# thunlp/OpenMatch

Hardware: NVIDIA H100
Metric: queries/sec top-1000 over 8.8M x 768 corpus (higher is better)
Workload: dtype f16

## Files before the change

### openmatch_b200/csrc/scan_epilogue.cuh

```cuda
#pragma once
#include <cuda_fp16.h>
#include <string.h>

#include <type_traits>

#include "gemm.cuh"

namespace om {

__host__ __device__ __forceinline__ uint32_t f32_orderable(float s) {
  s = s + 0.0f;
#ifdef __CUDA_ARCH__
  uint32_t u = __float_as_uint(s);
#else
  uint32_t u;
  memcpy(&u, &s, 4);
#endif
  return (u & 0x80000000u) ? ~u : (u | 0x80000000u);
}
__host__ __device__ __forceinline__ float f32_from_orderable(uint32_t u) {
  u = (u & 0x80000000u) ? (u & 0x7fffffffu) : ~u;
#ifdef __CUDA_ARCH__
  return __uint_as_float(u);
#else
  float s;
  memcpy(&s, &u, 4);
  return s;
#endif
}
__host__ __device__ __forceinline__ unsigned long long make_key(float s, uint32_t row) {
  return (static_cast<unsigned long long>(f32_orderable(s)) << 32) | static_cast<unsigned long long>(0xffffffffu - row);
}
__host__ __device__ __forceinline__ uint32_t key_row(unsigned long long k) {
  return 0xffffffffu - static_cast<uint32_t>(k & 0xffffffffull);
}
__host__ __device__ __forceinline__ float key_score(unsigned long long k) {
  return f32_from_orderable(static_cast<uint32_t>(k >> 32));
}

constexpr int kStashThreads = 32 * kGemmEpiWarps;

template <int N>
using SurvivorMask = std::conditional_t<N == 64, unsigned long long, uint32_t>;
__device__ __forceinline__ int mask_popc(uint32_t m) { return __popc(m); }
__device__ __forceinline__ int mask_popc(unsigned long long m) { return __popcll(m); }
__device__ __forceinline__ int mask_ffs(uint32_t m) { return __ffs(m); }
__device__ __forceinline__ int mask_ffs(unsigned long long m) { return __ffsll(static_cast<long long>(m)); }

template <int N, int BIT = 1>
__device__ __forceinline__ float pick(const float (&v)[N], int i) {
  if constexpr (N == 1) {
    return v[0];
  } else {
    float a[N / 2];
#pragma unroll
    for (int j = 0; j < N / 2; ++j) a[j] = (i & BIT) ? v[2 * j + 1] : v[2 * j];
    return pick<N / 2, 2 * BIT>(a, i);
  }
}

template <int N>
__device__ __forceinline__ SurvivorMask<N> survivors(const float (&v)[N], float t) {
  float mx = fmaxf(v[0], v[1]);
#pragma unroll
  for (int i = 2; i < N; i += 2) mx = fmaxf(mx, fmaxf(v[i], v[i + 1]));
  if (!(mx > t)) return 0;
  SurvivorMask<N> mask = 0;
#pragma unroll
  for (int w = 0; w < N / 32; ++w) {
    uint32_t m = 0;
#pragma unroll
    for (int i = 0; i < 32; ++i) m |= (v[32 * w + i] > t ? 1u : 0u) << i;
    mask |= static_cast<SurvivorMask<N>>(m) << (32 * w);
  }
  return mask;
}

template <int S, int N, class Col>
__device__ __forceinline__ int park(const float (&v)[N], SurvivorMask<N> mask, Col col, int k, unsigned long long* stash,
                                    int row, unsigned long long* cand, int* count, int* overflow, int C,
                                    uint32_t row_base) {
  const int n = mask_popc(mask);
  int pos = 0;
  if (k + n > S) {
    pos = atomicAdd(count + row, k + n - S);
    if (pos + (k + n - S) > C) *overflow = 1;
  }
  unsigned long long* mine = cand + static_cast<size_t>(row) * C;
  int idx = k;
#pragma unroll 1
  while (mask) {
    const int i = mask_ffs(mask) - 1;
    mask &= mask - 1;
    const unsigned long long key = make_key(pick(v, i), row_base + static_cast<uint32_t>(col(i)));
    if (idx < S)
      stash[idx * kStashThreads] = key;
    else if (pos + idx - S < C)
      mine[pos + idx - S] = key;
    ++idx;
  }
  return idx < S ? idx : S;
}

template <int N, class Col>
__device__ __forceinline__ SurvivorMask<N> allowed(SurvivorMask<N> mask, const uint32_t* allow, uint32_t row_base, Col col) {
  SurvivorMask<N> keep = 0;
#pragma unroll 1
  while (mask) {
    const int i = mask_ffs(mask) - 1;
    const SurvivorMask<N> bit = static_cast<SurvivorMask<N>>(1) << i;
    mask &= ~bit;
    const uint32_t r = row_base + static_cast<uint32_t>(col(i));
    if ((__ldg(allow + (r >> 5)) >> (r & 31)) & 1u) keep |= bit;
  }
  return keep;
}

__device__ __forceinline__ void drain_stash(const unsigned long long* stash, int n, unsigned long long* list, int pos,
                                            int C, int* overflow) {
  for (int j = 0; j < n; ++j)
    if (pos + j < C) list[pos + j] = stash[j * kStashThreads];
  if (n > 0 && pos + n > C) *overflow = 1;
}

constexpr int kFragStash = 4;
constexpr int kFragStashBytes = 2 * 2 * kFragStash * kStashThreads * 8;

template <int COLS, bool ALLOW = false>
struct FragFilter {
  unsigned long long* stash;
  unsigned long long* cand;
  int* count;
  int* overflow;
  int C;
  uint32_t row_base;
  int lane;
  const uint32_t* allow = nullptr;
  int buf = 0;
  int p_n[2] = {0, 0}, p_excl[2] = {0, 0}, p_pos[2] = {0, 0}, p_row = 0, p_buf = 0;

  __device__ __forceinline__ int col(int i) const { return 8 * (i >> 1) + 2 * (lane & 3) + (i & 1); }

  template <int H>
  __device__ __forceinline__ int filter_row(const float (&acc)[2 * COLS], float t, int row, int col0, int lim,
                                            unsigned long long* sb) const {
    float v[COLS];
#pragma unroll
    for (int i = 0; i < COLS; ++i) v[i] = acc[4 * (i >> 1) + 2 * H + (i & 1)];
    SurvivorMask<COLS> mask = survivors(v, t);
    if (!mask) return 0;
    if (lim < 4 * COLS) {
#pragma unroll 1
      for (int i = 0; i < COLS; ++i)
        if (col(i) >= lim) mask &= ~(static_cast<SurvivorMask<COLS>>(1) << i);
    }
    if constexpr (ALLOW) mask = allowed<COLS>(mask, allow, row_base, [&](int i) { return col0 + col(i); });
    return park<kFragStash>(v, mask, [&](int i) { return col0 + col(i); }, 0, sb, row, cand, count, overflow, C,
                            row_base);
  }

  __device__ __forceinline__ void drain() {
    if (!__any_sync(0xffffffffu, (p_n[0] | p_n[1]) != 0)) return;
    const unsigned long long* s = stash + p_buf * (2 * kFragStash * kStashThreads);
#pragma unroll
    for (int h = 0; h < 2; ++h)
      drain_stash(s + h * kFragStash * kStashThreads, p_n[h], cand + static_cast<size_t>(p_row + 8 * h) * C,
                  __shfl_sync(0xffffffffu, p_pos[h], lane & ~3) + p_excl[h], C, overflow);
    p_n[0] = p_n[1] = 0;
  }

  __device__ __forceinline__ void tile(const float (&acc)[2 * COLS], float t0, float t1, int row0, int col0, int n_cols) {
    drain();
    const int lim = n_cols - col0;
    unsigned long long* sb = stash + buf * (2 * kFragStash * kStashThreads);
    const int k[2] = {filter_row<0>(acc, t0, row0, col0, lim, sb),
                      filter_row<1>(acc, t1, row0 + 8, col0, lim, sb + kFragStash * kStashThreads)};
    if (!__any_sync(0xffffffffu, (k[0] | k[1]) != 0)) return;
#pragma unroll
    for (int h = 0; h < 2; ++h) {
      int x = k[h];
      int y = __shfl_up_sync(0xffffffffu, x, 1, 4);
      if ((lane & 3) >= 1) x += y;
      y = __shfl_up_sync(0xffffffffu, x, 2, 4);
      if ((lane & 3) >= 2) x += y;
      const int n = __shfl_sync(0xffffffffu, x, lane | 3);
      if ((lane & 3) == 0 && n > 0) p_pos[h] = atomicAdd(count + row0 + 8 * h, n);
      p_n[h] = k[h];
      p_excl[h] = x - k[h];
    }
    p_row = row0;
    p_buf = buf;
    buf ^= 1;
  }
};

template <bool ALLOW>
struct ScanAllow {};
template <>
struct ScanAllow<true> {
  const uint32_t* allow;
};
template <bool DENSE, bool ALLOW = false>
struct EpiScan : ScanAllow<ALLOW> {
  static_assert(!(DENSE && ALLOW), "a filtered first round runs as a threshold round at -inf");
  const float* thr;
  unsigned long long* cand;
  int* count;
  int* overflow;
  int nq, n_cols, C;
  uint32_t row_base;
  static constexpr bool kPrefetch = false;
  static constexpr int kStash = 8;
  __host__ __device__ static constexpr int smem_bytes(int) { return DENSE ? 0 : 2 * kStash * kStashThreads * 8; }
  struct State {
    float t;
    int k, tid, buf;
    unsigned long long* stash;
    int p_n, p_pos, p_row, p_buf;
  };
  __device__ __forceinline__ void bind(State& s, uint8_t* smem, int epi_tid) const {
    s.stash = reinterpret_cast<unsigned long long*>(smem);
    s.tid = epi_tid;
    s.buf = 0;
    s.p_n = 0;
  }
  __device__ __forceinline__ void finish(State& s) const { drain(s); }
  __device__ __forceinline__ void begin(State& s, int row, int, int) const {
    s.t = (row < nq && !DENSE) ? thr[row] : __int_as_float(0x7f800000);
    s.k = 0;
    if constexpr (DENSE) {
      s.p_n = 0;
      s.buf = 0;
    }
  }
  __device__ __forceinline__ unsigned long long* slot0(const State& s, int buf) const {
    return s.stash + static_cast<size_t>(buf) * kStash * kStashThreads + s.tid;
  }
  __device__ __forceinline__ void drain(State& s) const {
    if (s.p_n > 0) {
      drain_stash(slot0(s, s.p_buf), s.p_n, cand + static_cast<size_t>(s.p_row) * C, s.p_pos, C, overflow);
      s.p_n = 0;
    }
  }
  __device__ __forceinline__ void end(State& s, int row) const {
    if constexpr (DENSE) return;
    drain(s);
    if (s.k > 0) {
      s.p_pos = atomicAdd(count + row, s.k);
      s.p_n = s.k;
      s.p_row = row;
      s.p_buf = s.buf;
      s.buf ^= 1;
    }
  }
  __device__ __forceinline__ void chunk(State& s, int row, int col0, const float (&v)[32]) const {
    if (row >= nq || col0 >= n_cols) return;
    if constexpr (DENSE) {
      unsigned long long* mine = cand + static_cast<size_t>(row) * C;
      if (col0 + 32 <= n_cols) {
#pragma unroll
        for (int i = 0; i < 32; i += 2) {
          ulonglong2 kk;
          kk.x = make_key(v[i], row_base + col0 + i);
          kk.y = make_key(v[i + 1], row_base + col0 + i + 1);
          *reinterpret_cast<ulonglong2*>(mine + col0 + i) = kk;
        }
      } else {
#pragma unroll
        for (int i = 0; i < 32; ++i)
          if (col0 + i < n_cols) mine[col0 + i] = make_key(v[i], row_base + col0 + i);
      }
      return;
    }
    uint32_t mask = survivors(v, s.t);
    if (!mask) return;
    const int lim = n_cols - col0;
    if (lim < 32) mask &= (1u << lim) - 1u;
    if constexpr (ALLOW) mask = allowed<32>(mask, this->allow, row_base + col0, [](int i) { return i; });
    s.k = park<kStash>(v, mask, [&](int i) { return col0 + i; }, s.k, slot0(s, s.buf), row, cand, count, overflow, C,
                       row_base);
  }
};

static inline cudaError_t launch_scan_core(bool dense, const uint32_t* allow, const __half* Q, int64_t ldq, const __half* X,
                                           int64_t ldx, int nq, int n_cols, int K, const float* thr,
                                           unsigned long long* cand, int* count, int* overflow, int C, uint32_t row_base,
                                           int num_sms, cudaStream_t stream) {
  auto launch = [&](const auto& epi) {
    return launch_gemm<128, 3, true, std::decay_t<decltype(epi)>, true>(Q, ldq, X, ldx, nq, n_cols, K, epi, num_sms, stream,
                                                                       true);
  };
  if (dense) return launch(EpiScan<true>{{}, thr, cand, count, overflow, nq, n_cols, C, row_base});
  if (allow) return launch(EpiScan<false, true>{{allow}, thr, cand, count, overflow, nq, n_cols, C, row_base});
  return launch(EpiScan<false>{{}, thr, cand, count, overflow, nq, n_cols, C, row_base});
}

}
```

### openmatch_b200/csrc/scan_gemm.cuh

```cuda
#pragma once
#include <cuda_fp16.h>

#include <type_traits>

#include "scan_epilogue.cuh"

namespace om {

constexpr int kScanBlockN = 256;
constexpr int kScanStages = 3;
constexpr int kScanABytes = kBlockM * kBlockK * 2;
constexpr int kScanBBytes = kScanBlockN * kBlockK * 2;
constexpr int kScanStageBytes = kScanABytes + kScanBBytes;
constexpr int kScanConsumers = kStashThreads;
constexpr int kScanStashOffset = kScanStages * kScanStageBytes;
constexpr int kScanBarOffset = kScanStashOffset + kFragStashBytes;
constexpr int kScanSmemBytes = kScanBarOffset + 2 * kScanStages * 8 + 1024;
static_assert(kScanSmemBytes <= 232448, "scan ring + stash exceed the 227 KB of shared memory an H100 block may use");

template <int CQ, int CX>
struct ScanCluster {
  static_assert((CQ == 2 || CQ == 4) && (CX == 1 || CX == 2), "scan cluster shapes: CQ in {2, 4}, CX in {1, 2}");
  static constexpr int kSize = CQ * CX;
  static constexpr int kShare = CQ + CX - 1;
  static constexpr int kQRows = kBlockM / CX;
  static constexpr int kXRows = kScanBlockN / CQ;
  static constexpr int kEmptyArrivals = kShare * (kScanConsumers / 32);
  __device__ static uint32_t peer_rank(uint32_t rank, int j) {
    const uint32_t a = rank % CQ, b = rank / CQ;
    if (j < CQ - 1) {
      const uint32_t o = static_cast<uint32_t>(j);
      return (o < a ? o : o + 1) + CQ * b;
    }
    const uint32_t o = static_cast<uint32_t>(j - (CQ - 1));
    return a + CQ * (o < b ? o : o + 1);
  }
  __device__ static uint16_t q_mask(uint32_t rank) {
    uint32_t m = 0;
#pragma unroll
    for (int b = 0; b < CX; ++b) m |= 1u << (rank % CQ + CQ * b);
    return static_cast<uint16_t>(m);
  }
  __device__ static uint16_t x_mask(uint32_t rank) {
    return static_cast<uint16_t>(((1u << CQ) - 1u) << (CQ * (rank / CQ)));
  }
};

template <int CQ, int CX, bool ALLOW>
__global__ void __launch_bounds__(kGemmProducerThreads + kScanConsumers, 1)
scan_wide_kernel(const __grid_constant__ CUtensorMap tmQ, const __grid_constant__ CUtensorMap tmX, int K,
                 const float* __restrict__ thr, unsigned long long* cand, int* count, int* overflow, int nq, int n_cols,
                 int C, uint32_t row_base, const uint32_t* __restrict__ allow) {
  using Cl = ScanCluster<CQ, CX>;
  extern __shared__ uint8_t smem_raw[];
  uint8_t* smem = reinterpret_cast<uint8_t*>((reinterpret_cast<uintptr_t>(smem_raw) + 1023) & ~uintptr_t(1023));
  unsigned long long* stash = reinterpret_cast<unsigned long long*>(smem + kScanStashOffset);
  uint64_t* full_bar = reinterpret_cast<uint64_t*>(smem + kScanBarOffset);
  uint64_t* empty_bar = full_bar + kScanStages;
  const uint32_t rank = cluster_ctarank();
  const int qa = static_cast<int>(rank % CQ), xb = static_cast<int>(rank / CQ);
  const int warp = __shfl_sync(0xffffffffu, static_cast<int>(threadIdx.x >> 5), 0);
  const int lane = static_cast<int>(threadIdx.x & 31);

  if (warp == 0 && lane == 0) {
    tma_prefetch_desc(&tmQ);
    tma_prefetch_desc(&tmX);
  }
  if (warp == 1 && lane == 0) {
    ring_init(full_bar, empty_bar, kScanStages, Cl::kEmptyArrivals);
    fence_barrier_init();
  }
  cluster_sync_all();

  const int qgroups = (nq + CQ * kBlockM - 1) / (CQ * kBlockM);
  const int num_tiles = qgroups * ((n_cols + CX * kScanBlockN - 1) / (CX * kScanBlockN));
  const int num_k = (K + kBlockK - 1) / kBlockK;

  if (warp < 4) {
    setmaxnreg_dec<40>();
    if (warp == 0 && lane == 0) {
      const uint16_t qmask = Cl::q_mask(rank), xmask = Cl::x_mask(rank);
      Ring<kScanStages> ring;
      for (int tile = static_cast<int>(cluster_id_x()); tile < num_tiles; tile += static_cast<int>(cluster_count_x())) {
        const int m_blk = (tile % qgroups) * CQ + qa;
        const int n_blk = (tile / qgroups) * CX + xb;
        for (int kb = 0; kb < num_k; ++kb) {
          uint64_t* bar = ring_acquire_tx(full_bar, empty_bar, ring, kScanStageBytes, 30);
          uint8_t* sa = smem + ring.stage * kScanStageBytes;
          if constexpr (CX == 1)
            tma_load_2d(sa, &tmQ, bar, kb * kBlockK, m_blk * kBlockM);
          else
            tma_load_2d_multicast(sa + xb * (Cl::kQRows * kBlockK * 2), &tmQ, bar, kb * kBlockK,
                                  m_blk * kBlockM + xb * Cl::kQRows, qmask);
          tma_load_2d_multicast(sa + kScanABytes + qa * (Cl::kXRows * kBlockK * 2), &tmX, bar, kb * kBlockK,
                                n_blk * kScanBlockN + qa * Cl::kXRows, xmask);
          ring.advance();
        }
      }
    }
  } else {
    setmaxnreg_inc<232>();
    const int et = static_cast<int>(threadIdx.x) - kGemmProducerThreads;
    const int wg = et >> 7;
    const int frow = 64 * wg + 16 * (warp & 3) + (lane >> 2);
    Ring<kScanStages> ring;
    FragFilter<64, ALLOW> filter{stash + et, cand, count, overflow, C, row_base, lane, allow};

    uint32_t peers[Cl::kShare - 1];
#pragma unroll
    for (int j = 0; j < Cl::kShare - 1; ++j) peers[j] = Cl::peer_rank(rank, j);
    auto release = [&](uint32_t s) {
      if (lane == 0) {
        mbar_arrive(&empty_bar[s]);
#pragma unroll
        for (int j = 0; j < Cl::kShare - 1; ++j) mbar_arrive_remote(&empty_bar[s], peers[j]);
      }
    };

    for (int tile = static_cast<int>(cluster_id_x()); tile < num_tiles; tile += static_cast<int>(cluster_count_x())) {
      const int m_blk = (tile % qgroups) * CQ + qa;
      const int n_blk = (tile / qgroups) * CX + xb;
      const int row0 = m_blk * kBlockM + frow, row1 = row0 + 8;
      const int col0 = n_blk * kScanBlockN;
      const float inf = __int_as_float(0x7f800000);
      const float t0 = row0 < nq ? thr[row0] : inf, t1 = row1 < nq ? thr[row1] : inf;

      float acc[128];
#pragma unroll
      for (int i = 0; i < 128; ++i) acc[i] = 0.f;
      ring_consume(
          full_bar, ring, 0, num_k, 31,
          [&](uint32_t stage, uint32_t accumulate) {
            const uint32_t a_addr = smem_u32(smem + stage * kScanStageBytes) + wg * (64 * 128);
            const uint32_t b_addr = smem_u32(smem + stage * kScanStageBytes + kScanABytes);
#pragma unroll
            for (int k = 0; k < kBlockK / kWgmmaK; ++k)
              wgmma_m64n256k16_f16<0, 0>(acc, wgmma_desc(a_addr + k * 32, kDescKMajorSW128),
                                         wgmma_desc(b_addr + k * 32, kDescKMajorSW128), (accumulate | k) != 0 ? 1u : 0u);
          },
          release);
      wgmma_fence_regs(acc);

      filter.tile(acc, t0, t1, row0, col0, n_cols);
    }
    filter.drain();
  }

  __syncthreads();
  cluster_sync_all();
}

template <int CQ, int CX, bool ALLOW>
static inline cudaError_t scan_wide_max_clusters(int num_sms, int* out) {
  static int max_clusters = -1;
  if (max_clusters < 0) {
    constexpr int kSize = ScanCluster<CQ, CX>::kSize;
    cudaError_t e =
        cudaFuncSetAttribute(scan_wide_kernel<CQ, CX, ALLOW>, cudaFuncAttributeMaxDynamicSharedMemorySize, kScanSmemBytes);
    if (e != cudaSuccess) return e;
    cudaLaunchConfig_t cfg = {};
    cfg.gridDim = dim3(kSize * (num_sms / kSize));
    cfg.blockDim = dim3(kGemmProducerThreads + kScanConsumers);
    cfg.dynamicSmemBytes = kScanSmemBytes;
    cudaLaunchAttribute attr[1];
    attr[0].id = cudaLaunchAttributeClusterDimension;
    attr[0].val.clusterDim = {static_cast<unsigned>(kSize), 1, 1};
    cfg.attrs = attr;
    cfg.numAttrs = 1;
    int n = 0;
    e = cudaOccupancyMaxActiveClusters(&n, scan_wide_kernel<CQ, CX, ALLOW>, &cfg);
    if (e != cudaSuccess) return e;
    max_clusters = n < num_sms / kSize ? n : num_sms / kSize;
  }
  *out = max_clusters;
  return cudaSuccess;
}

template <int CQ, int CX, bool ALLOW>
static inline cudaError_t launch_scan_wide(const __half* Q, int64_t ldq, const __half* X, int64_t ldx, int nq, int n_cols,
                                           int K, const float* thr, unsigned long long* cand, int* count, int* overflow,
                                           int C, uint32_t row_base, const uint32_t* allow, int num_sms,
                                           cudaStream_t stream, int* max_clusters_out) {
  using Cl = ScanCluster<CQ, CX>;
  CUtensorMap tmQ, tmX;
  if (make_tmap_bf16_2d(&tmQ, Q, (uint64_t)K, (uint64_t)nq, (uint64_t)ldq * 2, kBlockK, Cl::kQRows) != 0)
    return cudaErrorInvalidValue;
  if (make_tmap_bf16_2d(&tmX, X, (uint64_t)K, (uint64_t)n_cols, (uint64_t)ldx * 2, kBlockK, Cl::kXRows) != 0)
    return cudaErrorInvalidValue;
  int max_clusters = 0;
  cudaError_t e = scan_wide_max_clusters<CQ, CX, ALLOW>(num_sms, &max_clusters);
  if (e != cudaSuccess) return e;
  *max_clusters_out = max_clusters;
  if (max_clusters < 1) return cudaErrorNotSupported;
  cudaLaunchConfig_t cfg = {};
  cfg.blockDim = dim3(kGemmProducerThreads + kScanConsumers);
  cfg.dynamicSmemBytes = kScanSmemBytes;
  cfg.stream = stream;
  cudaLaunchAttribute attr[1];
  attr[0].id = cudaLaunchAttributeClusterDimension;
  attr[0].val.clusterDim = {static_cast<unsigned>(Cl::kSize), 1, 1};
  cfg.attrs = attr;
  cfg.numAttrs = 1;
  const int qgroups = (nq + CQ * kBlockM - 1) / (CQ * kBlockM);
  const int64_t num_tiles = static_cast<int64_t>(qgroups) * ((n_cols + CX * kScanBlockN - 1) / (CX * kScanBlockN));
  const int clusters = num_tiles < max_clusters ? static_cast<int>(num_tiles) : max_clusters;
  cfg.gridDim = dim3(Cl::kSize * clusters);
  return cudaLaunchKernelEx(&cfg, scan_wide_kernel<CQ, CX, ALLOW>, tmQ, tmX, K, thr, cand, count, overflow, nq, n_cols, C,
                            row_base, allow);
}

static inline cudaError_t launch_scan_cluster(int cq, int cx, const __half* Q, int64_t ldq, const __half* X, int64_t ldx,
                                              int nq, int n_cols, int K, const float* thr, unsigned long long* cand,
                                              int* count, int* overflow, int C, uint32_t row_base, const uint32_t* allow,
                                              int num_sms, cudaStream_t stream, int* max_clusters) {
  *max_clusters = 0;
  if (nq <= 0 || n_cols <= 0 || K <= 0) return cudaSuccess;
  auto launch = [&](auto cq_c, auto cx_c) {
    constexpr int CQ = decltype(cq_c)::value, CX = decltype(cx_c)::value;
    return allow ? launch_scan_wide<CQ, CX, true>(Q, ldq, X, ldx, nq, n_cols, K, thr, cand, count, overflow, C, row_base,
                                                  allow, num_sms, stream, max_clusters)
                 : launch_scan_wide<CQ, CX, false>(Q, ldq, X, ldx, nq, n_cols, K, thr, cand, count, overflow, C, row_base,
                                                   nullptr, num_sms, stream, max_clusters);
  };
  using I1 = std::integral_constant<int, 1>;
  using I2 = std::integral_constant<int, 2>;
  using I4 = std::integral_constant<int, 4>;
  if (cq == 2 && cx == 1) return launch(I2{}, I1{});
  if (cq == 4 && cx == 1) return launch(I4{}, I1{});
  if (cq == 2 && cx == 2) return launch(I2{}, I2{});
  if (cq == 4 && cx == 2) return launch(I4{}, I2{});
  return cudaErrorInvalidValue;
}

}
```

Measured before the change: 38530.

## Widen scan tile to 384 columns with split n256+n128 wgmma

Raises the corpus-side tile width from 256 to 384 columns. Each k-step now issues an m64n256 plus an m64n128 wgmma, sharing the A descriptor, and the fragment filter is split into parts of 64 and 32 columns. This is meant to reuse each loaded query tile across more corpus rows and cut the per-tile epilogue and barrier overhead. In exchange the accumulator grows to 192 registers per thread, which risks spills given the 232-register cap, and the larger B stage increases the shared memory each stage needs.

Result: faster. 39360, median of 6 (+2.1%).

```diff
diff --git a/openmatch_b200/csrc/scan_epilogue.cuh b/openmatch_b200/csrc/scan_epilogue.cuh
--- a/openmatch_b200/csrc/scan_epilogue.cuh
+++ b/openmatch_b200/csrc/scan_epilogue.cuh
@@ -141,22 +141,34 @@
 
   __device__ __forceinline__ int col(int i) const { return 8 * (i >> 1) + 2 * (lane & 3) + (i & 1); }
 
+  template <int H, int OFF, int N>
+  __device__ __forceinline__ int filter_part(const float (&acc)[2 * COLS], float t, int row, int col0, int lim,
+                                             unsigned long long* sb, int k) const {
+    float v[N];
+#pragma unroll
+    for (int i = 0; i < N; ++i) v[i] = acc[4 * ((OFF + i) >> 1) + 2 * H + (i & 1)];
+    SurvivorMask<N> mask = survivors(v, t);
+    if (!mask) return k;
+    if (lim < 4 * COLS) {
+#pragma unroll 1
+      for (int i = 0; i < N; ++i)
+        if (col(OFF + i) >= lim) mask &= ~(static_cast<SurvivorMask<N>>(1) << i);
+    }
+    if constexpr (ALLOW) mask = allowed<N>(mask, allow, row_base, [&](int i) { return col0 + col(OFF + i); });
+    return park<kFragStash>(v, mask, [&](int i) { return col0 + col(OFF + i); }, k, sb, row, cand, count, overflow, C,
+                            row_base);
+  }
+
   template <int H>
   __device__ __forceinline__ int filter_row(const float (&acc)[2 * COLS], float t, int row, int col0, int lim,
                                             unsigned long long* sb) const {
-    float v[COLS];
-#pragma unroll
-    for (int i = 0; i < COLS; ++i) v[i] = acc[4 * (i >> 1) + 2 * H + (i & 1)];
-    SurvivorMask<COLS> mask = survivors(v, t);
-    if (!mask) return 0;
-    if (lim < 4 * COLS) {
-#pragma unroll 1
-      for (int i = 0; i < COLS; ++i)
-        if (col(i) >= lim) mask &= ~(static_cast<SurvivorMask<COLS>>(1) << i);
-    }
-    if constexpr (ALLOW) mask = allowed<COLS>(mask, allow, row_base, [&](int i) { return col0 + col(i); });
-    return park<kFragStash>(v, mask, [&](int i) { return col0 + col(i); }, 0, sb, row, cand, count, overflow, C,
-                            row_base);
+    static_assert(COLS == 32 || COLS == 64 || COLS == 96, "a row is one part of 32 or 64 values, or 64 + 32");
+    if constexpr (COLS <= 64) {
+      return filter_part<H, 0, COLS>(acc, t, row, col0, lim, sb, 0);
+    } else {
+      const int k = filter_part<H, 0, 64>(acc, t, row, col0, lim, sb, 0);
+      return filter_part<H, 64, COLS - 64>(acc, t, row, col0, lim, sb, k);
+    }
   }
 
   __device__ __forceinline__ void drain() {
diff --git a/openmatch_b200/csrc/scan_gemm.cuh b/openmatch_b200/csrc/scan_gemm.cuh
--- a/openmatch_b200/csrc/scan_gemm.cuh
+++ b/openmatch_b200/csrc/scan_gemm.cuh
@@ -7,7 +7,7 @@
 
 namespace om {
 
-constexpr int kScanBlockN = 256;
+constexpr int kScanBlockN = 384;
 constexpr int kScanStages = 3;
 constexpr int kScanABytes = kBlockM * kBlockK * 2;
 constexpr int kScanBBytes = kScanBlockN * kBlockK * 2;
@@ -104,7 +104,7 @@
     const int wg = et >> 7;
     const int frow = 64 * wg + 16 * (warp & 3) + (lane >> 2);
     Ring<kScanStages> ring;
-    FragFilter<64, ALLOW> filter{stash + et, cand, count, overflow, C, row_base, lane, allow};
+    FragFilter<kScanBlockN / 4, ALLOW> filter{stash + et, cand, count, overflow, C, row_base, lane, allow};
 
     uint32_t peers[Cl::kShare - 1];
 #pragma unroll
@@ -125,18 +125,23 @@
       const float inf = __int_as_float(0x7f800000);
       const float t0 = row0 < nq ? thr[row0] : inf, t1 = row1 < nq ? thr[row1] : inf;
 
-      float acc[128];
-#pragma unroll
-      for (int i = 0; i < 128; ++i) acc[i] = 0.f;
+      float acc[192];
+      float(&acc_lo)[128] = *reinterpret_cast<float(*)[128]>(acc);
+      float(&acc_hi)[64] = *reinterpret_cast<float(*)[64]>(acc + 128);
+#pragma unroll
+      for (int i = 0; i < 192; ++i) acc[i] = 0.f;
       ring_consume(
           full_bar, ring, 0, num_k, 31,
           [&](uint32_t stage, uint32_t accumulate) {
             const uint32_t a_addr = smem_u32(smem + stage * kScanStageBytes) + wg * (64 * 128);
             const uint32_t b_addr = smem_u32(smem + stage * kScanStageBytes + kScanABytes);
 #pragma unroll
-            for (int k = 0; k < kBlockK / kWgmmaK; ++k)
-              wgmma_m64n256k16_f16<0, 0>(acc, wgmma_desc(a_addr + k * 32, kDescKMajorSW128),
-                                         wgmma_desc(b_addr + k * 32, kDescKMajorSW128), (accumulate | k) != 0 ? 1u : 0u);
+            for (int k = 0; k < kBlockK / kWgmmaK; ++k) {
+              const uint64_t da = wgmma_desc(a_addr + k * 32, kDescKMajorSW128);
+              const uint32_t acc_k = (accumulate | k) != 0 ? 1u : 0u;
+              wgmma_m64n256k16_f16<0, 0>(acc_lo, da, wgmma_desc(b_addr + k * 32, kDescKMajorSW128), acc_k);
+              wgmma_m64n128k16_f16<0, 0>(acc_hi, da, wgmma_desc(b_addr + 256 * 128 + k * 32, kDescKMajorSW128), acc_k);
+            }
           },
           release);
       wgmma_fence_regs(acc);
```
